# Spandan7724/Audio-Watermarking-Deep-Learning-Watermarks-for-Authenticating-Speech

Hardware: AMD Instinct MI355X
Metric: 1-s@16kHz clips/sec (gen+det+loss fwd-bwd) (higher is better)
Workload: dtype f32; 1 GPU; main16 train step: Generator+Detector+6 losses fwd-bwd + Adam, B=256 clips/GPU x 1 GPU, 1-s @ 16 kHz, message_bits=16 (BASELINE configs[2]); batch_per_gpu=256, global_batch=256, clip_len=16000, optimizer=fused flat Adam (wm_adam_step), parallelism=single

## Files before the change

audio-watermarking-deep-learning-watermarks-for-authenticating-speech_amd/csrc/losses.hip:

```cpp
#include "wm_common.hpp"
using namespace wm;

namespace {

__device__ __forceinline__ int mod_small(int idx, int n, float inv_n) {
    int q = (int)((float)idx * inv_n);
    int r = idx - q * n;
    if (r < 0) r += n;
    if (r >= n) r -= n;
    return r;
}

__global__ __launch_bounds__(256) void bce_fwd_kernel(const float* __restrict__ logits, const long long* __restrict__ message,
                                                      int B, int R, int T, int NO, float* __restrict__ partial) {
    __shared__ float scratch[8];
    const int r = blockIdx.y, per_clip = T * NO;
    const float inv = 1.0f / (float)NO;
    const long long msg = (r < B) ? message[r] : 0;
    const float yl = r < B ? 1.f : 0.f;
    const float* lp = logits + (size_t)r * per_clip;
    float sl = 0.f, sb = 0.f;
#pragma unroll 4
    for (int k = 0; k < 16; ++k) {
        const int idx = blockIdx.x * 4096 + k * 256 + threadIdx.x;
// ... 30 lines not shown
            float d;
            if (o == 0) d = bce_logits_grad(x, yl, kl);
            else d = (r < B) ? bce_logits_grad(x, (float)((msg >> (o - 1)) & 1), kb) : 0.f;
            dp[idx] = d;
        }
    }
}

__global__ __launch_bounds__(256) void abs_sum_kernel(const float* __restrict__ x, size_t n, float* __restrict__ partial) {
    __shared__ float scratch[4];
    float s = 0.f;
    for (size_t i = (size_t)blockIdx.x * 256 + threadIdx.x; i < n; i += (size_t)gridDim.x * 256) s += fabsf(x[i]);
    s = block_sum<4>(s, scratch);
    if (threadIdx.x == 0) partial[blockIdx.x] = s;
}

__global__ void l1_bwd_kernel(const float* __restrict__ x, const float* __restrict__ g, size_t n, float* __restrict__ dx) {
    const size_t i = (size_t)blockIdx.x * blockDim.x + threadIdx.x;
    if (i >= n) return;
    const float k = g[0] / (float)n, v = x[i];
    dx[i] = v > 0.f ? k : (v < 0.f ? -k : 0.f);
}

__global__ __launch_bounds__(256) void sum_scale2_kernel(const float* __restrict__ partial, int n, double scale, float* out) {
    __shared__ double scratch[4];
    double s = 0.0;
    for (int i = threadIdx.x; i < n; i += 256) s += (double)partial[i];
    s = block_sum_d<4>(s, scratch);
    if (threadIdx.x == 0) out[0] = (float)(s * scale);
}

__global__ void adam_kernel(float* __restrict__ p, const float* __restrict__ g, float* __restrict__ m, float* __restrict__ v,
                            size_t n, float step_size, float b1, float b2, float eps, float bc2_sqrt) {
    const size_t i = (size_t)blockIdx.x * blockDim.x + threadIdx.x;
    if (i >= n) return;
    const float gi = g[i];
    const float mi = fmaf(b1, m[i], (1.f - b1) * gi);
    const float vi = fmaf(b2, v[i], (1.f - b2) * gi * gi);
    m[i] = mi; v[i] = vi;
    const float denom = sqrtf(vi) / bc2_sqrt + eps;
    p[i] -= step_size * (mi / denom);
}

}

namespace wm {
int launch_sum_scale2(const float* partial, int n, double scale, float* out, hipStream_t stream) {
    hipLaunchKernelGGL(sum_scale2_kernel, dim3(1), dim3(256), 0, stream, partial, n, scale, out);
    WM_CHECK_LAUNCH();
    return 0;
}
}

extern "C" {

int wm_bce_fwd(const float* logits, const long long* message, float* partial, float* loc_out, float* bce_out, int B, int R,
               int T, int NO, hipStream_t stream) {
    if ((long long)T * NO >= (1 << 23) || R <= 0 || R > 65535) return (int)hipErrorInvalidValue;
    const int chunks = (T * NO + 4095) / 4096, grid = chunks * R;
    hipLaunchKernelGGL(bce_fwd_kernel, dim3(chunks, R), dim3(256), 0, stream, logits, message, B, R, T, NO, partial);
    WM_CHECK_LAUNCH();
    hipLaunchKernelGGL(sum_scale2_kernel, dim3(1), dim3(256), 0, stream, (const float*)partial, grid, 1.0 / ((double)R * T), loc_out);
    WM_CHECK_LAUNCH();
    if (NO > 1) {
        hipLaunchKernelGGL(sum_scale2_kernel, dim3(1), dim3(256), 0, stream, (const float*)partial + grid, grid,
                           1.0 / ((double)B * T * (NO - 1)), bce_out);
        WM_CHECK_LAUNCH();
    }
    return 0;
}

int wm_bce_bwd(const float* logits, const long long* message, const float* g_loc, const float* g_bce, float* dlogits, int B,
               int R, int T, int NO, hipStream_t stream) {
    if ((long long)T * NO >= (1 << 23) || R <= 0 || R > 65535) return (int)hipErrorInvalidValue;
    hipLaunchKernelGGL(bce_bwd_kernel, dim3((T * NO + 4095) / 4096, R), dim3(256), 0, stream, logits, message, g_loc, g_bce, B, R, T,
                       NO, dlogits);
    WM_CHECK_LAUNCH();
    return 0;
}

int wm_l1_fwd(const float* x, float* partial, float* out, long long n, hipStream_t stream) {
    const int grid = 256;
    hipLaunchKernelGGL(abs_sum_kernel, dim3(grid), dim3(256), 0, stream, x, (size_t)n, partial);
    WM_CHECK_LAUNCH();
    hipLaunchKernelGGL(sum_scale2_kernel, dim3(1), dim3(256), 0, stream, (const float*)partial, grid, 1.0 / (double)n, out);
    WM_CHECK_LAUNCH();
    return 0;
}

int wm_l1_bwd(const float* x, const float* g, float* dx, long long n, hipStream_t stream) {
    hipLaunchKernelGGL(l1_bwd_kernel, dim3((unsigned)((n + 255) / 256)), dim3(256), 0, stream, x, g, (size_t)n, dx);
    WM_CHECK_LAUNCH();
    return 0;
}

int wm_adam_step(float* p, const float* g, float* m, float* v, long long n, double lr, double beta1, double beta2, double eps,
                 int step, hipStream_t stream) {
    if (step < 1 || n < 0) return (int)hipErrorInvalidValue;
    if (n == 0) return 0;
    const double bc1 = 1.0 - pow(beta1, (double)step);
    const double bc2s = sqrt(1.0 - pow(beta2, (double)step));
    hipLaunchKernelGGL(adam_kernel, dim3((unsigned)((n + 255) / 256)), dim3(256), 0, stream, p, g, m, v, (size_t)n,
                       (float)(lr / bc1), (float)beta1, (float)beta2, (float)eps, (float)bc2s);
    WM_CHECK_LAUNCH();
    return 0;
}

}
// ... 1 lines not shown
```

audio-watermarking-deep-learning-watermarks-for-authenticating-speech_amd/csrc/lstm.hip:

```cpp
#include "wm_common.hpp"
#include <type_traits>
using namespace wm;

namespace {

#ifdef WM_STAMP
__device__ unsigned long long* g_lstm_stamp = nullptr;
#define LSTAMP(var, val) unsigned long long var; asm volatile("s_memtime %0\n\ts_waitcnt lgkmcnt(0)" : "=s"(var), "+v"(val))
#define LSTAMP_ACC(i, a, b) tm[i] += (b) - (a)
#else
#define LSTAMP(var, val)
#define LSTAMP_ACC(i, a, b)
#endif

__device__ __forceinline__ int gate_row(int np) { return (np & 3) * 64 + (np >> 2); }

typedef float v2f __attribute__((ext_vector_type(2)));
template <int K>
__device__ __forceinline__ float quad_bcast(float v) {
    constexpr int ctrl = K | (K << 2) | (K << 4) | (K << 6);
    return __int_as_float(__builtin_amdgcn_update_dpp(0, __float_as_int(v), ctrl, 0xf, 0xf, false));
}

__global__ __launch_bounds__(256) void lstm_xproj_kernel(const float* __restrict__ x, const float* __restrict__ w_ih,
// ... 1292 lines not shown
            }
        }
        __syncthreads();
        if (next < ntiles) write_tile(next);
        __syncthreads();
        tile = next;
    }
    float* out = partial + (size_t)blockIdx.x * (256 * 128 + 256);
#pragma unroll
    for (int mt = 0; mt < 2; ++mt)
#pragma unroll
        for (int nt = 0; nt < 4; ++nt)
#pragma unroll
            for (int r = 0; r < 16; ++r)
                out[(wave * 64 + mt * 32 + mfma_row(r, half)) * 128 + nt * 32 + l31] = acc[mt][nt][r];
    float* red = reinterpret_cast<float*>(smem_raw);
    __syncthreads();
#pragma unroll
    for (int e = 0; e < 4; ++e) red[(tid >> 6) * 256 + 4 * (tid & 63) + e] = bs[e];
    __syncthreads();
    out[256 * 128 + tid] = (red[tid] + red[256 + tid]) + (red[512 + tid] + red[768 + tid]);
}

__global__ void lstm_wgrad_reduce_kernel(const float* __restrict__ partial, int nparts, float* dw_ih, float* dw_hh,
                                         float* db_ih, float* db_hh, int accumulate) {
    const int i = blockIdx.x * blockDim.x + threadIdx.x;
    constexpr int stride = 256 * 128 + 256;
    if (i >= stride) return;
    double sd = 0.0;
    for (int p = 0; p < nparts; ++p) sd += (double)partial[(size_t)p * stride + i];
    const float s = (float)sd;
    if (i < 256 * 128) {
        const int n = gate_row(i >> 7), j = i & 127;
        float* dst = (j < 64) ? dw_ih + n * 64 + j : dw_hh + n * 64 + (j - 64);
        *dst = accumulate ? *dst + s : s;
    } else {
        const int n = gate_row(i - 256 * 128);
        db_ih[n] = accumulate ? db_ih[n] + s : s;
        db_hh[n] = accumulate ? db_hh[n] + s : s;
    }
}

}

extern "C" {

#ifdef WM_STAMP
int wm_debug_set_lstm_stamp_buffer(unsigned long long* buf) {
    return (int)hipMemcpyToSymbol(HIP_SYMBOL(g_lstm_stamp), &buf, sizeof(buf));
}
#endif

int wm_lstm_xproj(const float* x, const float* w_ih, const float* b_ih, const float* b_hh, float* xp, int B, int T,
                  hipStream_t stream) {
    if (T & 3) return (int)hipErrorInvalidValue;
    hipLaunchKernelGGL(lstm_xproj_kernel, dim3(B * ((T + 127) / 128)), dim3(256), 0, stream, x, w_ih, b_ih, b_hh, xp, T);
    WM_CHECK_LAUNCH();
    return 0;
}

int wm_lstm_fwd(const float* xp, const float* w_hh, float* hout, float* gates, float* cst, int B, int T, hipStream_t stream) {
    if (T & 3) return (int)hipErrorInvalidValue;
    if (gates && cst) hipLaunchKernelGGL(lstm_fwd_kernel<true>, dim3(B), dim3(256), 0, stream, xp, w_hh, hout, gates, cst, T);
    else hipLaunchKernelGGL(lstm_fwd_kernel<false>, dim3(B), dim3(256), 0, stream, xp, w_hh, hout, gates, cst, T);
// ... 44 lines not shown
    constexpr size_t lds = (size_t)2 * 4 * 3 * 32 * 72 * 2 + (size_t)(4 * 64 * 33 + 4 * 64 + 2 * 64 * 4) * sizeof(float);
    static wm::DevOnce done;
    if (!wm::dev_done(done)) {
        WM_TRY(hipFuncSetAttribute(reinterpret_cast<const void*>(lstm_bwd_fused_kernel), hipFuncAttributeMaxDynamicSharedMemorySize, (int)lds));
        wm::dev_mark(done);
    }
    hipLaunchKernelGGL(lstm_bwd_fused_kernel, dim3(B), dim3(256), lds, stream, gates, cst, dh_out, w_hh, w_ih, dx, T);
    WM_CHECK_LAUNCH();
    return 0;
}

int wm_lstm_bwd_wgrad(float* gates, const float* cst, const float* dh_out, const float* w_hh, const float* x, const float* h,
                      float* partial, float* dw_ih, float* dw_hh, float* db_ih, float* db_hh, int B, int T, int accumulate,
                      hipStream_t stream) {
    if (B <= 0 || (T & 31) || T < 64) return (int)hipErrorInvalidValue;
    constexpr size_t lds = (size_t)(2 * 256 * 36 + 2 * 64 * 4) * sizeof(float);
    static wm::DevOnce done;
    if (!wm::dev_done(done)) {
        WM_TRY(hipFuncSetAttribute(reinterpret_cast<const void*>(lstm_bwd_ws_kernel), hipFuncAttributeMaxDynamicSharedMemorySize, (int)lds));
        wm::dev_mark(done);
    }
    hipLaunchKernelGGL(lstm_bwd_ws_kernel, dim3(B), dim3(512), lds, stream, gates, cst, dh_out, w_hh, x, h, partial, T);
    WM_CHECK_LAUNCH();
    constexpr int n = 256 * 128 + 256;
    hipLaunchKernelGGL(lstm_wgrad_reduce_kernel, dim3((n + 255) / 256), dim3(256), 0, stream, (const float*)partial, B,
                       dw_ih, dw_hh, db_ih, db_hh, accumulate);
    WM_CHECK_LAUNCH();
    return 0;
}

static int g_lstm_dx_bf = 1;
int wm_set_lstm_dx_bf16x6(int on, hipStream_t) { g_lstm_dx_bf = on ? 1 : 0; return 0; }

int wm_lstm_dx(const float* da, const float* w_ih, float* dx, int B, int T, hipStream_t stream) {
    const int ntiles = B * ((T + 63) / 64);
    if (g_lstm_dx_bf) {
        constexpr size_t ldsb = (size_t)3 * 64 * 264 * 2;
        static wm::DevOnce doneb;
        if (!wm::dev_done(doneb)) { WM_TRY(hipFuncSetAttribute(reinterpret_cast<const void*>(lstm_dx_bf_kernel), hipFuncAttributeMaxDynamicSharedMemorySize, (int)ldsb)); wm::dev_mark(doneb); }
        hipLaunchKernelGGL(lstm_dx_bf_kernel, dim3(ntiles < kNumCU ? ntiles : kNumCU), dim3(256), ldsb, stream, da, w_ih, dx, B, T);
        WM_CHECK_LAUNCH();
        return 0;
    }
    constexpr size_t lds = (size_t)(256 * 64 + 64 * 257) * sizeof(float);
    static wm::DevOnce done;
    if (!wm::dev_done(done)) { WM_TRY(hipFuncSetAttribute(reinterpret_cast<const void*>(lstm_dx_kernel), hipFuncAttributeMaxDynamicSharedMemorySize, (int)lds)); wm::dev_mark(done); }
    hipLaunchKernelGGL(lstm_dx_kernel, dim3(ntiles < kNumCU ? ntiles : kNumCU), dim3(256), lds, stream, da, w_ih, dx, B, T);
    WM_CHECK_LAUNCH();
    return 0;
}

int wm_lstm_wgrad(const float* da, const float* x, const float* h, float* partial, float* dw_ih, float* dw_hh,
                  float* db_ih, float* db_hh, int B, int T, int accumulate, hipStream_t stream) {
    int grid;
    if (g_lstm_dx_bf) {
        constexpr size_t ldsb = (size_t)(3 * 32 * 264 + 3 * 128 * 40) * 2;
        static wm::DevOnce doneb;
        if (!wm::dev_done(doneb)) { WM_TRY(hipFuncSetAttribute(reinterpret_cast<const void*>(lstm_wgrad_bf_kernel), hipFuncAttributeMaxDynamicSharedMemorySize, (int)ldsb)); wm::dev_mark(doneb); }
        const int ntiles = B * ((T + 31) / 32);
        grid = ntiles < kNumCU ? ntiles : kNumCU;
        hipLaunchKernelGGL(lstm_wgrad_bf_kernel, dim3(grid), dim3(256), ldsb, stream, da, x, h, partial, B, T);
    } else {
        constexpr size_t lds = (size_t)(64 * 256 + 128 * 67) * sizeof(float);
        static wm::DevOnce done;
        if (!wm::dev_done(done)) { WM_TRY(hipFuncSetAttribute(reinterpret_cast<const void*>(lstm_wgrad_kernel), hipFuncAttributeMaxDynamicSharedMemorySize, (int)lds)); wm::dev_mark(done); }
        const int ntiles = B * ((T + 63) / 64);
        grid = ntiles < kNumCU ? ntiles : kNumCU;
        hipLaunchKernelGGL(lstm_wgrad_kernel, dim3(grid), dim3(256), lds, stream, da, x, h, partial, B, T);
    }
    WM_CHECK_LAUNCH();
    constexpr int n = 256 * 128 + 256;
    hipLaunchKernelGGL(lstm_wgrad_reduce_kernel, dim3((n + 255) / 256), dim3(256), 0, stream, (const float*)partial, grid,
                       dw_ih, dw_hh, db_ih, db_hh, accumulate);
    WM_CHECK_LAUNCH();
    return 0;
}

}
```

audio-watermarking-deep-learning-watermarks-for-authenticating-speech_amd/csrc/postproc.hip:

```cpp
#include "wm_common.hpp"
using namespace wm;

namespace {

constexpr int kMaxTaps = 128;

__global__ __launch_bounds__(256) void postproc_fwd_kernel(const float* __restrict__ d_in, const float* __restrict__ taps,
                                                           int ntaps, float thr, float max_rms, float eps, int stages,
                                                           float* __restrict__ f_out, float* __restrict__ d_out,
                                                           float* __restrict__ stats, int T) {
    extern __shared__ __align__(16) float smem[];
    float* xs = smem;
    float* ks = smem + T + kMaxTaps;
    __shared__ float scratch[8];
    const int b = blockIdx.x, tid = threadIdx.x, pad = (ntaps - 1) / 2;
    const float* x = d_in + (size_t)b * T;
    const bool do_fir = stages & 1;
    for (int i = tid; i < T + 2 * pad; i += 256) {
        const int t = i - pad;
        xs[i] = (t >= 0 && t < T) ? x[t] : 0.f;
    }
    if (tid < ntaps) ks[tid] = taps[tid];
    __syncthreads();
    float ss = 0.f;
// ... 58 lines not shown
    }
    __syncthreads();
    for (int t = tid; t < T; t += 256) {
        float acc;
        if (stages & 1) {
            acc = 0.f;
            for (int j = 0; j < ntaps; ++j) acc = fmaf(ks[j], gs[t + 2 * pad - j], acc);
        } else {
            acc = gs[pad + t];
        }
        d_raw[(size_t)b * T + t] = acc;
    }
}

__global__ void embed_gather_kernel(const float* __restrict__ table, const long long* __restrict__ message,
                                    float* __restrict__ vec, int B, int nrows, int* __restrict__ err) {
    const int i = blockIdx.x * blockDim.x + threadIdx.x;
    if (i >= B * 64) return;
    const long long m = message[i >> 6];
    if (m < 0 || m >= nrows) { if (err) *err = 1; vec[i] = 0.f; return; }
    vec[i] = table[(size_t)m * 64 + (i & 63)];
}

__global__ void embed_scatter_add_kernel(float* __restrict__ dtable, const long long* __restrict__ message,
                                         const float* __restrict__ dvec, int B, int nrows) {
    const int d = threadIdx.x;
    if (d >= 64) return;
    for (int b = 0; b < B; ++b) {
        const long long m = message[b];
        if (m < 0 || m >= nrows) continue;
        dtable[(size_t)m * 64 + d] += dvec[(size_t)b * 64 + d];
    }
}

__global__ __launch_bounds__(256) void rowsum_kernel(const float* __restrict__ x, float* __restrict__ out, int T4) {
    __shared__ float scratch[4];
    const float4* xr = reinterpret_cast<const float4*>(x) + (size_t)blockIdx.x * T4;
    float s = 0.f;
    for (int i = threadIdx.x; i < T4; i += 256) { const float4 v = xr[i]; s += (v.x + v.y) + (v.z + v.w); }
    s = block_sum<4>(s, scratch);
    if (threadIdx.x == 0) out[blockIdx.x] = s;
}

}

extern "C" {

int wm_postproc_fwd(const float* d_in, const float* taps, int ntaps, float thr, float max_rms, float eps, int stages,
                    float* f_out, float* d_out, float* stats, int B, int T, hipStream_t stream) {
    if (ntaps < 1 || ntaps > kMaxTaps || !(ntaps & 1) || T > 36000) return (int)hipErrorInvalidValue;
    const size_t lds = (size_t)(T + 2 * kMaxTaps) * sizeof(float);
    static size_t lds_set = 0;
    if (lds > lds_set) {
        WM_TRY(hipFuncSetAttribute(reinterpret_cast<const void*>(postproc_fwd_kernel), hipFuncAttributeMaxDynamicSharedMemorySize, (int)lds));
        lds_set = lds;
// ... 6 lines not shown

int wm_postproc_bwd(const float* g, const float* f_in, const float* stats, const float* taps, int ntaps, float thr,
                    float max_rms, int stages, float* d_raw, int B, int T, hipStream_t stream) {
    if (ntaps < 1 || ntaps > kMaxTaps || !(ntaps & 1) || T > 36000) return (int)hipErrorInvalidValue;
    const size_t lds = (size_t)(T + 2 * kMaxTaps) * sizeof(float);
    static size_t lds_set = 0;
    if (lds > lds_set) {
        WM_TRY(hipFuncSetAttribute(reinterpret_cast<const void*>(postproc_bwd_kernel), hipFuncAttributeMaxDynamicSharedMemorySize, (int)lds));
        lds_set = lds;
    }
    hipLaunchKernelGGL(postproc_bwd_kernel, dim3(B), dim3(256), lds, stream, g, f_in, stats, taps, ntaps, thr, max_rms,
                       stages, d_raw, T);
    WM_CHECK_LAUNCH();
    return 0;
}

int wm_embed_gather(const float* table, const long long* message, float* vec, int B, int nrows, int* err, hipStream_t stream) {
    hipLaunchKernelGGL(embed_gather_kernel, dim3((B * 64 + 255) / 256), dim3(256), 0, stream, table, message, vec, B, nrows, err);
    WM_CHECK_LAUNCH();
    return 0;
}

int wm_embed_scatter_add(float* dtable, const long long* message, const float* dvec, int B, int nrows, hipStream_t stream) {
    hipLaunchKernelGGL(embed_scatter_add_kernel, dim3(1), dim3(64), 0, stream, dtable, message, dvec, B, nrows);
    WM_CHECK_LAUNCH();
    return 0;
}

int wm_rowsum(const float* x, float* out, int rows, int T, hipStream_t stream) {
    if (T & 3) return (int)hipErrorInvalidValue;
    hipLaunchKernelGGL(rowsum_kernel, dim3(rows), dim3(256), 0, stream, x, out, T / 4);
    WM_CHECK_LAUNCH();
    return 0;
}

}
```

audio-watermarking-deep-learning-watermarks-for-authenticating-speech_amd/csrc/small_convs.hip:

```cpp
#include "wm_common.hpp"
using namespace wm;

namespace {

__global__ __launch_bounds__(256) void stem_fwd_kernel(const float* __restrict__ s, const float* __restrict__ w,
                                                       const float* __restrict__ bias, float* __restrict__ y, int T) {
    __shared__ float ss[1024 + 8];
    __shared__ float ws[64 * 8];
    const int tilesPerClip = (T + 1023) / 1024;
    const int b = blockIdx.x / tilesPerClip, t0 = (blockIdx.x % tilesPerClip) * 1024;
    const float* sb = s + (size_t)b * T;
    for (int i = threadIdx.x; i < 1024 + 6; i += 256) {
        const int t = t0 - 3 + i;
        ss[i] = (t >= 0 && t < T) ? sb[t] : 0.f;
    }
    for (int i = threadIdx.x; i < 512; i += 256) {
        const int co = i >> 3, j = i & 7;
        ws[i] = (j < 7) ? w[co * 7 + j] : bias[co];
    }
    __syncthreads();
    const int t = t0 + 4 * threadIdx.x;
    if (t >= T) return;
    float v[10];
#pragma unroll
// ... 2 lines not shown
#pragma unroll 4
    for (int co = 0; co < 64; ++co) {
        const float* wc = ws + co * 8;
        float4 o = make_float4(wc[7], wc[7], wc[7], wc[7]);
#pragma unroll
        for (int j = 0; j < 7; ++j) {
            const float wj = wc[j];
            o.x = fmaf(wj, v[j], o.x);
            o.y = fmaf(wj, v[j + 1], o.y);
            o.z = fmaf(wj, v[j + 2], o.z);
            o.w = fmaf(wj, v[j + 3], o.w);
        }
        *reinterpret_cast<float4*>(yb + (size_t)co * T) = o;
    }
}

__global__ __launch_bounds__(256) void stem_bwd_kernel(const float* __restrict__ g, const float* __restrict__ s,
                                                       const float* __restrict__ w, float* __restrict__ ds,
                                                       float* __restrict__ partial, int B, int T, int nds) {
    constexpr int NT = 256, GS = NT + 8;
    extern __shared__ __align__(16) float smem[];
    float* gs = smem;
    float* ss = gs + 64 * GS;
    float* ws = ss + NT + 40;
    float* dsp = ws + 512;
    const int tid = threadIdx.x, lane = tid & 63, wave = tid >> 6, half = lane >> 5, l31 = lane & 31;
    for (int i = tid; i < 512; i += 256) ws[i] = ((i & 7) < 7) ? w[(i >> 3) * 7 + (i & 7)] : 0.f;
    const int tilesPerClip = (T + NT - 1) / NT, ntiles = B * tilesPerClip;
    f32x16 acc[2];
#pragma unroll
    for (int r = 0; r < 16; ++r) { acc[0][r] = 0.f; acc[1][r] = 0.f; }
    float4 sg[16];
    float hg[2], sv[2];
    auto load_piece = [&](int tile, int p) {
        const int b = tile / tilesPerClip, t0 = (tile % tilesPerClip) * NT;
        const float* gb = g + (size_t)b * 64 * T;
        if (p < 16) {
            const int i = tid + p * 256, c = i >> 6, q = i & 63;
            sg[p] = *reinterpret_cast<const float4*>(gb + (size_t)c * T + min(t0 + 4 * q, T - 4));
            return;
        }
#pragma unroll
        for (int k = 0; k < 2; ++k) {
            const int i = min(tid + k * 256, 64 * 6 - 1), c = i / 6, h = i % 6;
            const int t = (h < 3) ? t0 - 3 + h : t0 + NT + (h - 3);
            hg[k] = gb[(size_t)c * T + min(max(t, 0), T - 1)];
            const int ts_ = t0 - 3 + tid + k * 256;
            sv[k] = s[(size_t)b * T + min(max(ts_, 0), T - 1)];
        }
    };
// ... 26 lines not shown
    };
    int tile = blockIdx.x;
    if (tile < ntiles) load_tile(tile);
    __syncthreads();
    if (tile < ntiles) write_tile(tile);
    __syncthreads();
    while (tile < ntiles) {
        const int next = tile + gridDim.x, nextc = min(next, ntiles - 1);
        const int b = tile / tilesPerClip, t0 = (tile % tilesPerClip) * NT;
        {
            const float* ap = gs + l31 * GS + 4 + wave * 64 + half;
            const float* bp = ss + wave * 64 + half + l31;
            const bool tapcol = l31 < 7, onecol = l31 == 7;
#pragma unroll
            for (int k2 = 0; k2 < 32; ++k2) {
                if ((k2 & 1) == 0 || k2 == 31) load_piece(nextc, k2 == 31 ? 16 : k2 >> 1);
                const float sval = bp[2 * k2];
                const float bv = tapcol ? sval : (onecol ? 1.f : 0.f);
                acc[0] = mfma32(ap[2 * k2], bv, acc[0]);
                acc[1] = mfma32(ap[32 * GS + 2 * k2], bv, acc[1]);
            }
        }
        if (ds && b < nds) {
            const int cg = wave, tq = lane;
            float o0 = 0.f, o1 = 0.f, o2 = 0.f, o3 = 0.f;
#pragma unroll 4
            for (int cc = 0; cc < 16; ++cc) {
                const int co = cg * 16 + cc;
                const float4 ga = *reinterpret_cast<const float4*>(gs + co * GS + 4 * tq);
                const float4 gb4 = *reinterpret_cast<const float4*>(gs + co * GS + 4 * tq + 4);
                const float4 gc = *reinterpret_cast<const float4*>(gs + co * GS + 4 * tq + 8);
                const float4 w0 = *reinterpret_cast<const float4*>(ws + co * 8), w1 = *reinterpret_cast<const float4*>(ws + co * 8 + 4);
                const float gv[10] = {ga.y, ga.z, ga.w, gb4.x, gb4.y, gb4.z, gb4.w, gc.x, gc.y, gc.z};
                const float wj[7] = {w0.x, w0.y, w0.z, w0.w, w1.x, w1.y, w1.z};
#pragma unroll
                for (int j = 0; j < 7; ++j) {
                    o0 = fmaf(gv[6 - j], wj[j], o0); o1 = fmaf(gv[7 - j], wj[j], o1);
                    o2 = fmaf(gv[8 - j], wj[j], o2); o3 = fmaf(gv[9 - j], wj[j], o3);
                }
            }
            *reinterpret_cast<float4*>(dsp + cg * NT + 4 * tq) = make_float4(o0, o1, o2, o3);
        }
        __syncthreads();
        if (ds && b < nds) {
            const int t = t0 + tid;
            if (t < T) ds[(size_t)b * T + t] = (dsp[tid] + dsp[NT + tid]) + (dsp[2 * NT + tid] + dsp[3 * NT + tid]);
        }
        if (next < ntiles) write_tile(next);
        __syncthreads();
        tile = next;
    }
    float* red = gs;
    for (int wv = 0; wv < 4; ++wv) {
        if (wave == wv && l31 < 8) {
#pragma unroll
            for (int mt = 0; mt < 2; ++mt)
#pragma unroll
                for (int r = 0; r < 16; ++r) {
                    const int o = (mt * 32 + mfma_row(r, half)) * 8 + l31;
                    red[o] = (wv == 0) ? acc[mt][r] : red[o] + acc[mt][r];
                }
        }
        __syncthreads();
    }
    float* out = partial + (size_t)blockIdx.x * 512;
    for (int i = tid; i < 512; i += 256) out[i] = red[i];
}

__global__ __launch_bounds__(256) void reduce_partials_kernel(const float* __restrict__ partial, int nparts, int stride, int count,
                                                              float* __restrict__ out, int accumulate) {
    __shared__ double sq[4][64];
    const int il = threadIdx.x & 63, grp = threadIdx.x >> 6, i = blockIdx.x * 64 + il;
    const int per = (nparts + 3) / 4, p0 = grp * per, p1 = min(p0 + per, nparts);
    double s0 = 0.0, s1 = 0.0;
    if (i < count) {
        int p = p0;
        for (; p + 1 < p1; p += 2) {
            s0 += (double)partial[(size_t)p * stride + i];
            s1 += (double)partial[(size_t)(p + 1) * stride + i];
        }
        if (p < p1) s0 += (double)partial[(size_t)p * stride + i];
    }
    sq[grp][il] = s0 + s1;
    __syncthreads();
    if (grp == 0 && i < count) {
        const float s = (float)((sq[0][il] + sq[1][il]) + (sq[2][il] + sq[3][il]));
        out[i] = accumulate ? out[i] + s : s;
    }
}
__global__ void stem_reduce_kernel(const float* __restrict__ partial, int nparts, float* dw, float* db, int accumulate) {
    const int i = blockIdx.x * blockDim.x + threadIdx.x;
    if (i >= 512) return;
    double sd = 0.0;
    for (int p = 0; p < nparts; ++p) sd += (double)partial[(size_t)p * 512 + i];
    const float s = (float)sd;
    const int co = i >> 3, j = i & 7;
    float* dst = (j < 7) ? dw + co * 7 + j : db + co;
    *dst = accumulate ? *dst + s : s;
}

__global__ __launch_bounds__(256) void head1_fwd_kernel(const float* __restrict__ x, const float* __restrict__ w,
                                                        const float* __restrict__ bias, float* __restrict__ y, int T4,
                                                        int total4) {
    const int i = blockIdx.x * 256 + threadIdx.x;
    if (i >= total4) return;
    const int b = i / T4, q = i % T4;
    const float4* xb = reinterpret_cast<const float4*>(x) + (size_t)b * 64 * T4 + q;
    const float b0 = bias[0];
    float4 o = make_float4(b0, b0, b0, b0);
#pragma unroll 8
    for (int c = 0; c < 64; ++c) {
        const float4 v = xb[(size_t)c * T4];
        const float wc = w[c];
        o.x = fmaf(wc, v.x, o.x); o.y = fmaf(wc, v.y, o.y); o.z = fmaf(wc, v.z, o.z); o.w = fmaf(wc, v.w, o.w);
    }
    reinterpret_cast<float4*>(y)[i] = o;
}

// ... 336 lines not shown
                                 ((red[128 + tid] + red[160 + tid]) + (red[192 + tid] + red[224 + tid]));
        else
            out[NO * 64 + tid] = (red[tid] + red[64 + tid]) + (red[128 + tid] + red[192 + tid]);
    }
}

}

extern "C" {

int wm_stem_fwd(const float* s, const float* w, const float* bias, float* y, int B, int T, hipStream_t stream) {
    if (T & 3) return (int)hipErrorInvalidValue;
    hipLaunchKernelGGL(stem_fwd_kernel, dim3(B * ((T + 1023) / 1024)), dim3(256), 0, stream, s, w, bias, y, T);
    WM_CHECK_LAUNCH();
    return 0;
}

#ifndef WM_STEM_WGS_PER_CU
#define WM_STEM_WGS_PER_CU 2
#endif
int wm_stem_bwd(const float* g, const float* s, const float* w, float* ds, float* partial, float* dw, float* db, int B,
                int T, int nds, int accumulate, hipStream_t stream) {
    if (T & 3) return (int)hipErrorInvalidValue;
    constexpr size_t lds = (size_t)(64 * 264 + 296 + 512 + 4 * 256) * sizeof(float);
    static wm::DevOnce attr_done;
    if (!wm::dev_done(attr_done)) {
        WM_TRY(hipFuncSetAttribute(reinterpret_cast<const void*>(stem_bwd_kernel), hipFuncAttributeMaxDynamicSharedMemorySize, (int)lds));
        wm::dev_mark(attr_done);
    }
    const int ntiles = B * ((T + 255) / 256);
    const int grid = ntiles < WM_STEM_WGS_PER_CU * kNumCU ? ntiles : WM_STEM_WGS_PER_CU * kNumCU;
    hipLaunchKernelGGL(stem_bwd_kernel, dim3(grid), dim3(256), lds, stream, g, s, w, ds, partial, B, T, nds);
    WM_CHECK_LAUNCH();
    hipLaunchKernelGGL(stem_reduce_kernel, dim3(2), dim3(256), 0, stream, (const float*)partial, grid, dw, db, accumulate);
    WM_CHECK_LAUNCH();
    return 0;
}

int wm_head1_fwd(const float* x, const float* w, const float* bias, float* y, int B, int T, hipStream_t stream) {
    if (T & 3) return (int)hipErrorInvalidValue;
    const int total4 = B * (T / 4);
    hipLaunchKernelGGL(head1_fwd_kernel, dim3((total4 + 255) / 256), dim3(256), 0, stream, x, w, bias, y, T / 4, total4);
    WM_CHECK_LAUNCH();
    return 0;
}

int wm_head1_tail_fwd(const float* x, const float* y2, const float* scale, const float* shift, const float* w, const float* bias,
                      float* out, void* mask, float* y, int B, int T, hipStream_t stream) {
    if ((T & 3) || B <= 0 || !y2 || !out) return (int)hipErrorInvalidValue;
    const int T4 = T / 4, grid = B * ((T4 + 255) / 256);
    if (mask) hipLaunchKernelGGL(head1_tail_fwd_kernel<true>, dim3(grid), dim3(256), 0, stream, x, y2, scale, shift, out, (unsigned*)mask, w, bias, y, T4);
    else hipLaunchKernelGGL(head1_tail_fwd_kernel<false>, dim3(grid), dim3(256), 0, stream, x, y2, scale, shift, out, (unsigned*)nullptr, w, bias, y, T4);
    WM_CHECK_LAUNCH();
    return 0;
}

int wm_head1_bwd(const float* g, const float* x, const float* w, float* dx, float* partial, float* dw, float* db, int B,
// ... 135 lines not shown
```

audio-watermarking-deep-learning-watermarks-for-authenticating-speech_amd/csrc/stft_loss.hip:

```cpp
#include "wm_common.hpp"
using namespace wm;

namespace {

enum { MODE_MEL = 0, MODE_LOUD = 1, MODE_HF = 2 };

struct StftArgs {
    const float* a;
    const float* b;
    float* gframes;
    float* partial;
    const float* fb;
    const int* klo; const int* khi;
    const int* mlo;
    float gscale;
    float thresh;
    int kcut;
    int T, F, hop;
};

__device__ __forceinline__ float2 cmul(float2 a, float2 b) { return make_float2(a.x * b.x - a.y * b.y, a.x * b.y + a.y * b.x); }

template <int LOGN>
__device__ __forceinline__ void fft_dif(float2* z, const float2* tw, int tid) {
// ... 143 lines not shown
__global__ void ola_gather_kernel(const float* __restrict__ gframes, float* __restrict__ dsig, int N, int hop, int F,
                                  int T, int total, int accumulate) {
    const int i = blockIdx.x * blockDim.x + threadIdx.x;
    if (i >= total) return;
    const int b = i / T, t = i % T, half = N / 2;
    const float* gf = gframes + (size_t)b * F * N;
    int pos[3];
    int np = 0;
    pos[np++] = t + half;
    if (t >= 1 && t <= half) pos[np++] = half - t;
    if (t <= T - 2 && 2 * (T - 1) - t + half < T + N) { const int q = 2 * (T - 1) - t + half; if (q >= T + half) pos[np++] = q; }
    float acc = 0.f;
    for (int j = 0; j < np; ++j) {
        const int pp = pos[j];
        int f_hi = pp / hop;
        if (f_hi > F - 1) f_hi = F - 1;
        int f_lo = (pp - N + hop) / hop;
        if (pp - N + 1 <= 0) f_lo = 0;
        for (int f = f_lo; f <= f_hi; ++f) acc += gf[(size_t)f * N + (pp - f * hop)];
    }
    dsig[i] = accumulate ? dsig[i] + acc : acc;
}

__global__ __launch_bounds__(256) void sum_scale_kernel(const float* __restrict__ partial, int n, double scale, float* out) {
    __shared__ double scratch[4];
    double s = 0.0;
    for (int i = threadIdx.x; i < n; i += 256) s += (double)partial[i];
    s = block_sum_d<4>(s, scratch);
    if (threadIdx.x == 0) out[0] = (float)(s * scale);
}

template <int LOGN, int MODE>
int launch_stft(const StftArgs& p, int B, hipStream_t stream) {
    constexpr int N = 1 << LOGN, NB = N / 2 + 1;
    constexpr size_t lds = (size_t)(2 * N + N + 4 * NB + (MODE == MODE_MEL ? 2 * NB + 192 : 0)) * sizeof(float);
    const int units = (MODE == MODE_HF) ? (p.F + 1) / 2 : p.F;
    hipLaunchKernelGGL((stft_loss_kernel<LOGN, MODE>), dim3(B * units), dim3(256), lds, stream, p);
    WM_CHECK_LAUNCH();
    return 0;
}

}

extern "C" {

int wm_mel_loss(const float* clean, const float* wm, const float* fb, const int* klo, const int* khi, const int* mlo,
                float* gframes, float* partial, float* loss_out, float* dsig, int B, int T, hipStream_t stream) {
    const int N = 1024, hop = 256, F = 1 + T / hop;
    if (T <= N / 2) return (int)hipErrorInvalidValue;
    const double count = (double)B * 64.0 * F;
    StftArgs p{clean, wm, dsig ? gframes : nullptr, partial, fb, klo, khi, mlo, (float)(1.0 / count), 0.f, 0, T, F, hop};
    int rc = launch_stft<10, MODE_MEL>(p, B, stream);
    if (rc) return rc;
    hipLaunchKernelGGL(sum_scale_kernel, dim3(1), dim3(256), 0, stream, (const float*)partial, B * F, 1.0 / count, loss_out);
    WM_CHECK_LAUNCH();
    if (dsig) {
        hipLaunchKernelGGL(ola_gather_kernel, dim3((B * T + 255) / 256), dim3(256), 0, stream, (const float*)gframes, dsig, N, hop, F, T, B * T, 0);
        WM_CHECK_LAUNCH();
    }
    return 0;
}

int wm_loud_loss(const float* clean, const float* wm, float thresh, float* gframes, float* partial, float* loss_out,
                 float* dsig, int B, int T, hipStream_t stream) {
    const int N = 2048, hop = 512, F = 1 + T / hop;
    if (T <= N / 2) return (int)hipErrorInvalidValue;
    const double count = (double)B * (N / 2 + 1) * F;
    StftArgs p{clean, wm, dsig ? gframes : nullptr, partial, nullptr, nullptr, nullptr, nullptr, (float)(1.0 / count), thresh, 0, T, F, hop};
    int rc = launch_stft<11, MODE_LOUD>(p, B, stream);
    if (rc) return rc;
    hipLaunchKernelGGL(sum_scale_kernel, dim3(1), dim3(256), 0, stream, (const float*)partial, B * F, 1.0 / count, loss_out);
    WM_CHECK_LAUNCH();
    if (dsig) {
        hipLaunchKernelGGL(ola_gather_kernel, dim3((B * T + 255) / 256), dim3(256), 0, stream, (const float*)gframes, dsig, N, hop, F, T, B * T, 0);
        WM_CHECK_LAUNCH();
    }
    return 0;
}

int wm_hf_penalty(const float* delta, int kcut, float* gframes, float* partial, float* loss_out, float* dsig, int B, int T,
                  hipStream_t stream) {
    const int N = 512, hop = 128, F = 1 + T / hop;
    if (T <= N / 2) return (int)hipErrorInvalidValue;
    const double count = (double)B * (N / 2 + 1) * F;
    const int units = (F + 1) / 2;
    StftArgs p{delta, nullptr, dsig ? gframes : nullptr, partial, nullptr, nullptr, nullptr, nullptr, (float)(1.0 / count), 0.f, kcut, T, F, hop};
    int rc = launch_stft<9, MODE_HF>(p, B, stream);
    if (rc) return rc;
    hipLaunchKernelGGL(sum_scale_kernel, dim3(1), dim3(256), 0, stream, (const float*)partial, B * units, 1.0 / count, loss_out);
    WM_CHECK_LAUNCH();
    if (dsig) {
        hipLaunchKernelGGL(ola_gather_kernel, dim3((B * T + 255) / 256), dim3(256), 0, stream, (const float*)gframes, dsig, N, hop, F, T, B * T, 0);
        WM_CHECK_LAUNCH();
    }
    return 0;
}

}
```

audio-watermarking-deep-learning-watermarks-for-authenticating-speech_amd/csrc/wm_common.hpp:

```cpp
#pragma once
#include <hip/hip_runtime.h>
#include <stdint.h>
#include <atomic>

#define WM_CHECK_LAUNCH() do { hipError_t e_ = hipGetLastError(); if (e_ != hipSuccess) return (int)e_; } while (0)
#define WM_TRY(expr) do { hipError_t e_ = (expr); if (e_ != hipSuccess) return (int)e_; } while (0)

namespace wm {

struct DevOnce {
    std::atomic<unsigned long long> mask{0};
};
inline bool dev_done(const DevOnce& d) {
    int dev = 0;
    if (hipGetDevice(&dev) != hipSuccess) return false;
    return (d.mask.load(std::memory_order_acquire) >> (dev & 63)) & 1ull;
}
inline void dev_mark(DevOnce& d) {
    int dev = 0;
    if (hipGetDevice(&dev) != hipSuccess) return;
    d.mask.fetch_or(1ull << (dev & 63), std::memory_order_release);
}

typedef float f32x16 __attribute__((ext_vector_type(16)));
typedef float f32x4 __attribute__((ext_vector_type(4)));

constexpr int kWave = 64;
constexpr int kNumCU = 256;

__device__ __forceinline__ f32x16 mfma32(float a, float b, f32x16 c) {
    return __builtin_amdgcn_mfma_f32_32x32x2f32(a, b, c, 0, 0, 0);
}
__device__ __forceinline__ int mfma_row(int r, int half) { return (r & 3) + 8 * (r >> 2) + 4 * half; }

__device__ __forceinline__ float wave_sum(float v) {
#pragma unroll
    for (int o = 32; o > 0; o >>= 1) v += __shfl_xor(v, o);
    return v;
}
__device__ __forceinline__ float half_wave_sum(float v) {
#pragma unroll
    for (int o = 16; o > 0; o >>= 1) v += __shfl_xor(v, o);
    return v;
}
__device__ __forceinline__ float half_wave_transpose_sum32(float (&x)[32], int lane) {
#pragma unroll
    for (int s = 4; s >= 0; --s) {
        const int h = 1 << s;
        const bool up = (lane >> s) & 1;
// ... 29 lines not shown
template <int NW>
__device__ __forceinline__ float block_sum(float v, float* scratch) {
    v = wave_sum(v);
    const int lane = threadIdx.x & 63, w = threadIdx.x >> 6;
    __syncthreads();
    if (lane == 0) scratch[w] = v;
    __syncthreads();
    float r = 0.f;
#pragma unroll
    for (int i = 0; i < NW; ++i) r += scratch[i];
    return r;
}
template <int NW>
__device__ __forceinline__ double block_sum_d(double v, double* scratch) {
    v = wave_sum_d(v);
    const int lane = threadIdx.x & 63, w = threadIdx.x >> 6;
    __syncthreads();
    if (lane == 0) scratch[w] = v;
    __syncthreads();
    double r = 0.0;
#pragma unroll
    for (int i = 0; i < NW; ++i) r += scratch[i];
    return r;
}

__device__ __forceinline__ float sigmoidf_acc(float x) { return 1.0f / (1.0f + expf(-x)); }

__device__ __forceinline__ float softplus_neg_abs(float x) {
    const float u = __expf(-fabsf(x));
    return (u < 0.01f) ? u * fmaf(u, fmaf(u, 0.33333334f, -0.5f), 1.0f) : __logf(1.0f + u);
}
__device__ __forceinline__ float bce_logits(float x, float y) { return fmaxf(x, 0.f) - x * y + softplus_neg_abs(x); }
__device__ __forceinline__ float bce_logits_grad(float x, float y, float k) {
    const float sg = __builtin_amdgcn_rcpf(1.0f + __expf(-x));
    return k * (sg - y);
}

int launch_sum_scale2(const float* partial, int n, double scale, float* out, hipStream_t stream);

#ifndef WM_STREAM_NT
#define WM_STREAM_NT 1
#endif
__device__ __forceinline__ float4 stream_load(const float4* p) {
#if WM_STREAM_NT
    const f32x4 v = __builtin_nontemporal_load(reinterpret_cast<const f32x4*>(p));
    return make_float4(v.x, v.y, v.z, v.w);
// ... 81 lines not shown
```

Before: 5292 clips/s.

## Parallelize small reductions and embedding scatter-add across more threads

Widens the scalar loss reductions to 1024 threads with four-way unrolled accumulation. Rewrites the LSTM weight-gradient and stem reductions to split partials across several wave groups with a shared column-sum helper. Parallelizes the embedding scatter-add across batch rows using ballot-based owner election in place of a single serial 64-thread block. Also drops the stem weight LDS staging in favour of direct global reads of the weights. The aim is to cut latency in reduction and scatter kernels that were serialized, at the cost of more shared-memory synchronization and extra code.

```diff
diff --git a/audio-watermarking-deep-learning-watermarks-for-authenticating-speech_amd/csrc/losses.hip b/audio-watermarking-deep-learning-watermarks-for-authenticating-speech_amd/csrc/losses.hip
--- a/audio-watermarking-deep-learning-watermarks-for-authenticating-speech_amd/csrc/losses.hip
+++ b/audio-watermarking-deep-learning-watermarks-for-authenticating-speech_amd/csrc/losses.hip
@@ -76,11 +76,18 @@
     dx[i] = v > 0.f ? k : (v < 0.f ? -k : 0.f);
 }
 
-__global__ __launch_bounds__(256) void sum_scale2_kernel(const float* __restrict__ partial, int n, double scale, float* out) {
-    __shared__ double scratch[4];
-    double s = 0.0;
-    for (int i = threadIdx.x; i < n; i += 256) s += (double)partial[i];
-    s = block_sum_d<4>(s, scratch);
+__global__ __launch_bounds__(1024) void sum_scale2_kernel(const float* __restrict__ partial, int n, double scale, float* out) {
+    __shared__ double scratch[16];
+    double s0 = 0.0, s1 = 0.0, s2 = 0.0, s3 = 0.0;
+    int i = threadIdx.x;
+    for (; i + 3072 < n; i += 4096) {
+        const float v0 = partial[i], v1 = partial[i + 1024], v2 = partial[i + 2048], v3 = partial[i + 3072];
+        s0 += (double)v0; s1 += (double)v1; s2 += (double)v2; s3 += (double)v3;
+    }
+    if (i < n) s0 += (double)partial[i];
+    if (i + 1024 < n) s1 += (double)partial[i + 1024];
+    if (i + 2048 < n) s2 += (double)partial[i + 2048];
+    const double s = block_sum_d<16>((s0 + s1) + (s2 + s3), scratch);
     if (threadIdx.x == 0) out[0] = (float)(s * scale);
 }
 
@@ -100,7 +107,7 @@
 
 namespace wm {
 int launch_sum_scale2(const float* partial, int n, double scale, float* out, hipStream_t stream) {
-    hipLaunchKernelGGL(sum_scale2_kernel, dim3(1), dim3(256), 0, stream, partial, n, scale, out);
+    hipLaunchKernelGGL(sum_scale2_kernel, dim3(1), dim3(1024), 0, stream, partial, n, scale, out);
     WM_CHECK_LAUNCH();
     return 0;
 }
@@ -114,10 +121,10 @@
     const int chunks = (T * NO + 4095) / 4096, grid = chunks * R;
     hipLaunchKernelGGL(bce_fwd_kernel, dim3(chunks, R), dim3(256), 0, stream, logits, message, B, R, T, NO, partial);
     WM_CHECK_LAUNCH();
-    hipLaunchKernelGGL(sum_scale2_kernel, dim3(1), dim3(256), 0, stream, (const float*)partial, grid, 1.0 / ((double)R * T), loc_out);
+    hipLaunchKernelGGL(sum_scale2_kernel, dim3(1), dim3(1024), 0, stream, (const float*)partial, grid, 1.0 / ((double)R * T), loc_out);
     WM_CHECK_LAUNCH();
     if (NO > 1) {
-        hipLaunchKernelGGL(sum_scale2_kernel, dim3(1), dim3(256), 0, stream, (const float*)partial + grid, grid,
+        hipLaunchKernelGGL(sum_scale2_kernel, dim3(1), dim3(1024), 0, stream, (const float*)partial + grid, grid,
                            1.0 / ((double)B * T * (NO - 1)), bce_out);
         WM_CHECK_LAUNCH();
     }
@@ -137,7 +144,7 @@
     const int grid = 256;
     hipLaunchKernelGGL(abs_sum_kernel, dim3(grid), dim3(256), 0, stream, x, (size_t)n, partial);
     WM_CHECK_LAUNCH();
-    hipLaunchKernelGGL(sum_scale2_kernel, dim3(1), dim3(256), 0, stream, (const float*)partial, grid, 1.0 / (double)n, out);
+    hipLaunchKernelGGL(sum_scale2_kernel, dim3(1), dim3(1024), 0, stream, (const float*)partial, grid, 1.0 / (double)n, out);
     WM_CHECK_LAUNCH();
     return 0;
 }
diff --git a/audio-watermarking-deep-learning-watermarks-for-authenticating-speech_amd/csrc/lstm.hip b/audio-watermarking-deep-learning-watermarks-for-authenticating-speech_amd/csrc/lstm.hip
--- a/audio-watermarking-deep-learning-watermarks-for-authenticating-speech_amd/csrc/lstm.hip
+++ b/audio-watermarking-deep-learning-watermarks-for-authenticating-speech_amd/csrc/lstm.hip
@@ -1338,14 +1338,13 @@
     out[256 * 128 + tid] = (red[tid] + red[256 + tid]) + (red[512 + tid] + red[768 + tid]);
 }
 
-__global__ void lstm_wgrad_reduce_kernel(const float* __restrict__ partial, int nparts, float* dw_ih, float* dw_hh,
-                                         float* db_ih, float* db_hh, int accumulate) {
-    const int i = blockIdx.x * blockDim.x + threadIdx.x;
-    constexpr int stride = 256 * 128 + 256;
-    if (i >= stride) return;
-    double sd = 0.0;
-    for (int p = 0; p < nparts; ++p) sd += (double)partial[(size_t)p * stride + i];
-    const float s = (float)sd;
+constexpr int kWgradSlab = 256 * 128 + 256;
+__global__ __launch_bounds__(512) void lstm_wgrad_reduce_kernel(const float* __restrict__ partial, int nparts, float* dw_ih,
+                                                                float* dw_hh, float* db_ih, float* db_hh, int accumulate) {
+    __shared__ double sq[8][64];
+    const int i = blockIdx.x * 64 + (threadIdx.x & 63);
+    const float s = (float)column_sum_d<8>(partial, nparts, (size_t)kWgradSlab, i, true, sq);
+    if (threadIdx.x >= 64) return;
     if (i < 256 * 128) {
         const int n = gate_row(i >> 7), j = i & 127;
         float* dst = (j < 64) ? dw_ih + n * 64 + j : dw_hh + n * 64 + (j - 64);
@@ -1356,6 +1355,7 @@
         db_hh[n] = accumulate ? db_hh[n] + s : s;
     }
 }
+static_assert(kWgradSlab % 64 == 0, "lstm_wgrad_reduce_kernel: whole 64-column blocks");
 
 }
 
@@ -1446,8 +1446,7 @@
     }
     hipLaunchKernelGGL(lstm_bwd_ws_kernel, dim3(B), dim3(512), lds, stream, gates, cst, dh_out, w_hh, x, h, partial, T);
     WM_CHECK_LAUNCH();
-    constexpr int n = 256 * 128 + 256;
-    hipLaunchKernelGGL(lstm_wgrad_reduce_kernel, dim3((n + 255) / 256), dim3(256), 0, stream, (const float*)partial, B,
+    hipLaunchKernelGGL(lstm_wgrad_reduce_kernel, dim3(kWgradSlab / 64), dim3(512), 0, stream, (const float*)partial, B,
                        dw_ih, dw_hh, db_ih, db_hh, accumulate);
     WM_CHECK_LAUNCH();
     return 0;
@@ -1493,8 +1492,7 @@
         hipLaunchKernelGGL(lstm_wgrad_kernel, dim3(grid), dim3(256), lds, stream, da, x, h, partial, B, T);
     }
     WM_CHECK_LAUNCH();
-    constexpr int n = 256 * 128 + 256;
-    hipLaunchKernelGGL(lstm_wgrad_reduce_kernel, dim3((n + 255) / 256), dim3(256), 0, stream, (const float*)partial, grid,
+    hipLaunchKernelGGL(lstm_wgrad_reduce_kernel, dim3(kWgradSlab / 64), dim3(512), 0, stream, (const float*)partial, grid,
                        dw_ih, dw_hh, db_ih, db_hh, accumulate);
     WM_CHECK_LAUNCH();
     return 0;
diff --git a/audio-watermarking-deep-learning-watermarks-for-authenticating-speech_amd/csrc/postproc.hip b/audio-watermarking-deep-learning-watermarks-for-authenticating-speech_amd/csrc/postproc.hip
--- a/audio-watermarking-deep-learning-watermarks-for-authenticating-speech_amd/csrc/postproc.hip
+++ b/audio-watermarking-deep-learning-watermarks-for-authenticating-speech_amd/csrc/postproc.hip
@@ -104,15 +104,37 @@
     vec[i] = table[(size_t)m * 64 + (i & 63)];
 }
 
-__global__ void embed_scatter_add_kernel(float* __restrict__ dtable, const long long* __restrict__ message,
-                                         const float* __restrict__ dvec, int B, int nrows) {
-    const int d = threadIdx.x;
-    if (d >= 64) return;
-    for (int b = 0; b < B; ++b) {
-        const long long m = message[b];
-        if (m < 0 || m >= nrows) continue;
-        dtable[(size_t)m * 64 + d] += dvec[(size_t)b * 64 + d];
-    }
+__global__ __launch_bounds__(256) void embed_scatter_add_kernel(float* __restrict__ dtable, const long long* __restrict__ message,
+                                                                const float* __restrict__ dvec, int B, int nrows) {
+    const int lane = threadIdx.x & 63, b = blockIdx.x * 4 + (threadIdx.x >> 6);
+    if (b >= B) return;
+    const long long m = message[b];
+    if (m < 0 || m >= nrows) return;
+    float* row = dtable + (size_t)m * 64 + lane;
+    float acc = 0.f;
+    bool owner = false;
+    for (int k0 = 0; k0 < B; k0 += 64) {
+        const int idx = k0 + lane;
+        const long long id = idx < B ? message[idx] : -1;
+        unsigned long long hit = __ballot(id == m);
+        if (k0 + 64 <= b) {
+            if (hit) return;
+            continue;
+        }
+        if (!owner) {
+            const int sh = b - k0;
+            if (hit & ((1ull << sh) - 1ull)) return;
+            hit &= ~((1ull << sh) - 1ull);
+            acc = *row;
+            owner = true;
+        }
+        while (hit) {
+            const int j = __builtin_ctzll(hit);
+            hit &= hit - 1ull;
+            acc += dvec[(size_t)(k0 + j) * 64 + lane];
+        }
+    }
+    *row = acc;
 }
 
 __global__ __launch_bounds__(256) void rowsum_kernel(const float* __restrict__ x, float* __restrict__ out, int T4) {
@@ -165,7 +187,8 @@
 }
 
 int wm_embed_scatter_add(float* dtable, const long long* message, const float* dvec, int B, int nrows, hipStream_t stream) {
-    hipLaunchKernelGGL(embed_scatter_add_kernel, dim3(1), dim3(64), 0, stream, dtable, message, dvec, B, nrows);
+    if (B <= 0) return 0;
+    hipLaunchKernelGGL(embed_scatter_add_kernel, dim3((B + 3) / 4), dim3(256), 0, stream, dtable, message, dvec, B, nrows);
     WM_CHECK_LAUNCH();
     return 0;
 }
diff --git a/audio-watermarking-deep-learning-watermarks-for-authenticating-speech_amd/csrc/small_convs.hip b/audio-watermarking-deep-learning-watermarks-for-authenticating-speech_amd/csrc/small_convs.hip
--- a/audio-watermarking-deep-learning-watermarks-for-authenticating-speech_amd/csrc/small_convs.hip
+++ b/audio-watermarking-deep-learning-watermarks-for-authenticating-speech_amd/csrc/small_convs.hip
@@ -48,10 +48,8 @@
     extern __shared__ __align__(16) float smem[];
     float* gs = smem;
     float* ss = gs + 64 * GS;
-    float* ws = ss + NT + 40;
-    float* dsp = ws + 512;
+    float* dsp = ss + NT + 40;
     const int tid = threadIdx.x, lane = tid & 63, wave = tid >> 6, half = lane >> 5, l31 = lane & 31;
-    for (int i = tid; i < 512; i += 256) ws[i] = ((i & 7) < 7) ? w[(i >> 3) * 7 + (i & 7)] : 0.f;
     const int tilesPerClip = (T + NT - 1) / NT, ntiles = B * tilesPerClip;
     f32x16 acc[2];
 #pragma unroll
@@ -124,17 +122,17 @@
             }
         }
         if (ds && b < nds) {
-            const int cg = wave, tq = lane;
+            const int cg = __builtin_amdgcn_readfirstlane(wave), tq = lane;
             float o0 = 0.f, o1 = 0.f, o2 = 0.f, o3 = 0.f;
 #pragma unroll 4
             for (int cc = 0; cc < 16; ++cc) {
                 const int co = cg * 16 + cc;
-                const float4 ga = *reinterpret_cast<const float4*>(gs + co * GS + 4 * tq);
-                const float4 gb4 = *reinterpret_cast<const float4*>(gs + co * GS + 4 * tq + 4);
-                const float4 gc = *reinterpret_cast<const float4*>(gs + co * GS + 4 * tq + 8);
-                const float4 w0 = *reinterpret_cast<const float4*>(ws + co * 8), w1 = *reinterpret_cast<const float4*>(ws + co * 8 + 4);
+                const f32x4 ga = lds_read4(gs + co * GS + 4 * tq);
+                const f32x4 gb4 = lds_read4(gs + co * GS + 4 * tq + 4);
+                const f32x4 gc = lds_read4(gs + co * GS + 4 * tq + 8);
+                const float* wc = w + co * 7;
                 const float gv[10] = {ga.y, ga.z, ga.w, gb4.x, gb4.y, gb4.z, gb4.w, gc.x, gc.y, gc.z};
-                const float wj[7] = {w0.x, w0.y, w0.z, w0.w, w1.x, w1.y, w1.z};
+                const float wj[7] = {wc[0], wc[1], wc[2], wc[3], wc[4], wc[5], wc[6]};
 #pragma unroll
                 for (int j = 0; j < 7; ++j) {
                     o0 = fmaf(gv[6 - j], wj[j], o0); o1 = fmaf(gv[7 - j], wj[j], o1);
@@ -172,30 +170,16 @@
 __global__ __launch_bounds__(256) void reduce_partials_kernel(const float* __restrict__ partial, int nparts, int stride, int count,
                                                               float* __restrict__ out, int accumulate) {
     __shared__ double sq[4][64];
-    const int il = threadIdx.x & 63, grp = threadIdx.x >> 6, i = blockIdx.x * 64 + il;
-    const int per = (nparts + 3) / 4, p0 = grp * per, p1 = min(p0 + per, nparts);
-    double s0 = 0.0, s1 = 0.0;
-    if (i < count) {
-        int p = p0;
-        for (; p + 1 < p1; p += 2) {
-            s0 += (double)partial[(size_t)p * stride + i];
-            s1 += (double)partial[(size_t)(p + 1) * stride + i];
-        }
-        if (p < p1) s0 += (double)partial[(size_t)p * stride + i];
-    }
-    sq[grp][il] = s0 + s1;
-    __syncthreads();
-    if (grp == 0 && i < count) {
-        const float s = (float)((sq[0][il] + sq[1][il]) + (sq[2][il] + sq[3][il]));
-        out[i] = accumulate ? out[i] + s : s;
-    }
-}
-__global__ void stem_reduce_kernel(const float* __restrict__ partial, int nparts, float* dw, float* db, int accumulate) {
-    const int i = blockIdx.x * blockDim.x + threadIdx.x;
-    if (i >= 512) return;
-    double sd = 0.0;
-    for (int p = 0; p < nparts; ++p) sd += (double)partial[(size_t)p * 512 + i];
-    const float s = (float)sd;
+    const int i = blockIdx.x * 64 + (threadIdx.x & 63);
+    const float s = (float)column_sum_d<4>(partial, nparts, (size_t)stride, i, i < count, sq);
+    if (threadIdx.x < 64 && i < count) out[i] = accumulate ? out[i] + s : s;
+}
+__global__ __launch_bounds__(1024) void stem_reduce_kernel(const float* __restrict__ partial, int nparts, float* dw, float* db,
+                                                           int accumulate) {
+    __shared__ double sq[16][64];
+    const int i = blockIdx.x * 64 + (threadIdx.x & 63);
+    const float s = (float)column_sum_d<16>(partial, nparts, (size_t)512, i, true, sq);
+    if (threadIdx.x >= 64) return;
     const int co = i >> 3, j = i & 7;
     float* dst = (j < 7) ? dw + co * 7 + j : db + co;
     *dst = accumulate ? *dst + s : s;
@@ -578,7 +562,7 @@
 int wm_stem_bwd(const float* g, const float* s, const float* w, float* ds, float* partial, float* dw, float* db, int B,
                 int T, int nds, int accumulate, hipStream_t stream) {
     if (T & 3) return (int)hipErrorInvalidValue;
-    constexpr size_t lds = (size_t)(64 * 264 + 296 + 512 + 4 * 256) * sizeof(float);
+    constexpr size_t lds = (size_t)(64 * 264 + 296 + 4 * 256) * sizeof(float);
     static wm::DevOnce attr_done;
     if (!wm::dev_done(attr_done)) {
         WM_TRY(hipFuncSetAttribute(reinterpret_cast<const void*>(stem_bwd_kernel), hipFuncAttributeMaxDynamicSharedMemorySize, (int)lds));
@@ -588,7 +572,7 @@
     const int grid = ntiles < WM_STEM_WGS_PER_CU * kNumCU ? ntiles : WM_STEM_WGS_PER_CU * kNumCU;
     hipLaunchKernelGGL(stem_bwd_kernel, dim3(grid), dim3(256), lds, stream, g, s, w, ds, partial, B, T, nds);
     WM_CHECK_LAUNCH();
-    hipLaunchKernelGGL(stem_reduce_kernel, dim3(2), dim3(256), 0, stream, (const float*)partial, grid, dw, db, accumulate);
+    hipLaunchKernelGGL(stem_reduce_kernel, dim3(8), dim3(1024), 0, stream, (const float*)partial, grid, dw, db, accumulate);
     WM_CHECK_LAUNCH();
     return 0;
 }
diff --git a/audio-watermarking-deep-learning-watermarks-for-authenticating-speech_amd/csrc/stft_loss.hip b/audio-watermarking-deep-learning-watermarks-for-authenticating-speech_amd/csrc/stft_loss.hip
--- a/audio-watermarking-deep-learning-watermarks-for-authenticating-speech_amd/csrc/stft_loss.hip
+++ b/audio-watermarking-deep-learning-watermarks-for-authenticating-speech_amd/csrc/stft_loss.hip
@@ -189,14 +189,6 @@
     dsig[i] = accumulate ? dsig[i] + acc : acc;
 }
 
-__global__ __launch_bounds__(256) void sum_scale_kernel(const float* __restrict__ partial, int n, double scale, float* out) {
-    __shared__ double scratch[4];
-    double s = 0.0;
-    for (int i = threadIdx.x; i < n; i += 256) s += (double)partial[i];
-    s = block_sum_d<4>(s, scratch);
-    if (threadIdx.x == 0) out[0] = (float)(s * scale);
-}
-
 template <int LOGN, int MODE>
 int launch_stft(const StftArgs& p, int B, hipStream_t stream) {
     constexpr int N = 1 << LOGN, NB = N / 2 + 1;
@@ -219,8 +211,8 @@
     StftArgs p{clean, wm, dsig ? gframes : nullptr, partial, fb, klo, khi, mlo, (float)(1.0 / count), 0.f, 0, T, F, hop};
     int rc = launch_stft<10, MODE_MEL>(p, B, stream);
     if (rc) return rc;
-    hipLaunchKernelGGL(sum_scale_kernel, dim3(1), dim3(256), 0, stream, (const float*)partial, B * F, 1.0 / count, loss_out);
-    WM_CHECK_LAUNCH();
+    rc = wm::launch_sum_scale2(partial, B * F, 1.0 / count, loss_out, stream);
+    if (rc) return rc;
     if (dsig) {
         hipLaunchKernelGGL(ola_gather_kernel, dim3((B * T + 255) / 256), dim3(256), 0, stream, (const float*)gframes, dsig, N, hop, F, T, B * T, 0);
         WM_CHECK_LAUNCH();
@@ -236,8 +228,8 @@
     StftArgs p{clean, wm, dsig ? gframes : nullptr, partial, nullptr, nullptr, nullptr, nullptr, (float)(1.0 / count), thresh, 0, T, F, hop};
     int rc = launch_stft<11, MODE_LOUD>(p, B, stream);
     if (rc) return rc;
-    hipLaunchKernelGGL(sum_scale_kernel, dim3(1), dim3(256), 0, stream, (const float*)partial, B * F, 1.0 / count, loss_out);
-    WM_CHECK_LAUNCH();
+    rc = wm::launch_sum_scale2(partial, B * F, 1.0 / count, loss_out, stream);
+    if (rc) return rc;
     if (dsig) {
         hipLaunchKernelGGL(ola_gather_kernel, dim3((B * T + 255) / 256), dim3(256), 0, stream, (const float*)gframes, dsig, N, hop, F, T, B * T, 0);
         WM_CHECK_LAUNCH();
@@ -254,8 +246,8 @@
     StftArgs p{delta, nullptr, dsig ? gframes : nullptr, partial, nullptr, nullptr, nullptr, nullptr, (float)(1.0 / count), 0.f, kcut, T, F, hop};
     int rc = launch_stft<9, MODE_HF>(p, B, stream);
     if (rc) return rc;
-    hipLaunchKernelGGL(sum_scale_kernel, dim3(1), dim3(256), 0, stream, (const float*)partial, B * units, 1.0 / count, loss_out);
-    WM_CHECK_LAUNCH();
+    rc = wm::launch_sum_scale2(partial, B * units, 1.0 / count, loss_out, stream);
+    if (rc) return rc;
     if (dsig) {
         hipLaunchKernelGGL(ola_gather_kernel, dim3((B * T + 255) / 256), dim3(256), 0, stream, (const float*)gframes, dsig, N, hop, F, T, B * T, 0);
         WM_CHECK_LAUNCH();
diff --git a/audio-watermarking-deep-learning-watermarks-for-authenticating-speech_amd/csrc/wm_common.hpp b/audio-watermarking-deep-learning-watermarks-for-authenticating-speech_amd/csrc/wm_common.hpp
--- a/audio-watermarking-deep-learning-watermarks-for-authenticating-speech_amd/csrc/wm_common.hpp
+++ b/audio-watermarking-deep-learning-watermarks-for-authenticating-speech_amd/csrc/wm_common.hpp
@@ -25,6 +25,9 @@
 typedef float f32x16 __attribute__((ext_vector_type(16)));
 typedef float f32x4 __attribute__((ext_vector_type(4)));
 
+typedef const volatile __attribute__((address_space(3))) f32x4 lds_f32x4_t;
+__device__ __forceinline__ f32x4 lds_read4(const float* p) { return *(lds_f32x4_t*)p; }
+
 constexpr int kWave = 64;
 constexpr int kNumCU = 256;
 
@@ -100,6 +103,34 @@
 #pragma unroll
     for (int i = 0; i < NW; ++i) r += scratch[i];
     return r;
+}
+
+template <int NG>
+__device__ __forceinline__ double column_sum_d(const float* __restrict__ partial, int nparts, size_t stride, int i, bool valid,
+                                               double (&sq)[NG][64]) {
+    const int il = threadIdx.x & 63, grp = threadIdx.x >> 6;
+    const int per = (nparts + NG - 1) / NG, p0 = grp * per, p1 = min(p0 + per, nparts);
+    double s0 = 0.0, s1 = 0.0, s2 = 0.0, s3 = 0.0;
+    if (valid) {
+        const float* col = partial + i;
+        int p = p0;
+        for (; p + 3 < p1; p += 4) {
+            const float v0 = col[(size_t)p * stride], v1 = col[(size_t)(p + 1) * stride];
+            const float v2 = col[(size_t)(p + 2) * stride], v3 = col[(size_t)(p + 3) * stride];
+            s0 += (double)v0; s1 += (double)v1; s2 += (double)v2; s3 += (double)v3;
+        }
+        if (p < p1) s0 += (double)col[(size_t)p * stride];
+        if (p + 1 < p1) s1 += (double)col[(size_t)(p + 1) * stride];
+        if (p + 2 < p1) s2 += (double)col[(size_t)(p + 2) * stride];
+    }
+    sq[grp][il] = (s0 + s1) + (s2 + s3);
+    __syncthreads();
+    double s = 0.0;
+    if (grp == 0) {
+#pragma unroll
+        for (int g = 0; g < NG; ++g) s += sq[g][il];
+    }
+    return s;
 }
 
 __device__ __forceinline__ float sigmoidf_acc(float x) { return 1.0f / (1.0f + expf(-x)); }
```

Measured after the change: 5365 clips/s, median of 6. +1.4%, better.
